# DoeringChristian/mitsuba3-experiments

Measured on AMD Instinct MI355X. Metric: Mpaths/sec on bedroom@1280×720 spp=256, 1/2/4/8 GPUs; HBM GB/s vs peak, higher is better.
Workload: dtype f32; 1 GPU; path-mis.py NEE+MIS (BASELINE configs[1]) on bedroom-proxy 1280x720, global spp=256 split over 1 rank(s) by sample range, max_depth=8, rr_depth=2; global_spp=256, spp_per_rank=256, parallelism=sample-range shards x1

## Files before the change

mitsuba3-experiments_amd/csrc/device_common.h:

```cpp
#pragma once
#include <hip/hip_runtime.h>

#include "mtx_core/bsdf.h"
#include "mtx_core/geometry.h"
#include "mtx_core/interaction.h"
#include "mtx_core/rng.h"
#include "wavefront.h"

namespace mtxd {

using namespace mtx;

inline size_t stack_bytes(const DevScene &s) {
  const size_t a = s.stack_entries, b = 2 * (size_t)s.occ_stack_entries;
  return (a > b ? a : b) * sizeof(uint32_t) * kTraceBlock;
}
inline size_t persistent_stack_bytes(const DevScene &s, bool occ) {
  return occ ? (size_t)s.occ_lds_entries * kTraceBlock * sizeof(uint2) + (size_t)s.occ_lds_top * 80
             : (size_t)s.lds_entries * kTraceBlock * sizeof(int32_t) + (size_t)s.lds_top * 64;
}

__device__ __forceinline__ SceneView make_view(const DevScene &s) {
  SceneView v;
  v.nodes = reinterpret_cast<const int32_t *>(s.nodes);
// ... 102 lines not shown
__device__ __forceinline__ uint32_t wave_append(uint32_t *counter, bool pred) {
  const uint64_t mask = __ballot(pred);
  const uint32_t prefix =
      __builtin_amdgcn_mbcnt_hi((uint32_t)(mask >> 32), __builtin_amdgcn_mbcnt_lo((uint32_t)mask, 0u));
  const uint32_t total = (uint32_t)__popcll(mask);
  uint32_t base = 0;
  if (total) {
    const uint32_t leader = (uint32_t)(__ffsll((unsigned long long)mask) - 1);
    if (lane_id() == leader) base = atomicAdd(counter, total);
    base = __builtin_amdgcn_readlane(base, leader);
  }
  return base + prefix;
}

template <int BLOCK>
__device__ __forceinline__ uint32_t block_reserve(uint32_t cnt, uint32_t *counter) {
  constexpr int W = BLOCK / 64;
  __shared__ uint32_t wsum[W];
  __shared__ uint32_t bbase;
  const uint32_t wave = threadIdx.x >> 6, lane = threadIdx.x & 63;
  uint32_t x = cnt;
#pragma unroll
  for (int off = 1; off < 64; off <<= 1) {
    const uint32_t y = __shfl_up(x, off);
    if (lane >= (uint32_t)off) x += y;
  }
  if (lane == 63) wsum[wave] = x;
  __syncthreads();
  if (threadIdx.x == 0) {
    uint32_t t = 0;
#pragma unroll
    for (int w = 0; w < W; ++w) {
      const uint32_t v = wsum[w];
      wsum[w] = t;
      t += v;
    }
    bbase = t ? atomicAdd(counter, t) : 0u;
  }
  __syncthreads();
  const uint32_t r = bbase + wsum[wave] + x - cnt;
  __syncthreads();
  return r;
}

template <int BLOCK>
__device__ __forceinline__ void block_append2(bool p0, bool p1, bool p1_hi, uint32_t *c, uint32_t parity,
                                              uint32_t &s0, uint32_t &s1) {
  constexpr int W = BLOCK / 64;
  __shared__ uint32_t wcnt[2][3][W];
  __shared__ uint32_t bbase[2][3];
  const uint32_t wave = threadIdx.x >> 6, lane = threadIdx.x & 63;
  const uint64_t m0 = __ballot(p0), ml = __ballot(p1 && !p1_hi), mh = __ballot(p1 && p1_hi);
  if (lane == 0) {
    wcnt[parity][0][wave] = (uint32_t)__popcll(m0);
    wcnt[parity][1][wave] = (uint32_t)__popcll(ml);
    wcnt[parity][2][wave] = (uint32_t)__popcll(mh);
  }
  __syncthreads();
  if (threadIdx.x == 0) {
    uint32_t t0 = 0, tl = 0, th = 0;
#pragma unroll
    for (int w = 0; w < W; ++w) {
      t0 += wcnt[parity][0][w];
      tl += wcnt[parity][1][w];
      th += wcnt[parity][2][w];
    }
    uint64_t base = 0;
    if (t0 | tl | th)
      base = atomicAdd(reinterpret_cast<unsigned long long *>(c), ((unsigned long long)(tl + th) << 32) | t0);
    bbase[parity][0] = (uint32_t)base;
    bbase[parity][1] = (uint32_t)(base >> 32);
    bbase[parity][2] = (uint32_t)(base >> 32) + tl;
  }
  __syncthreads();
  uint32_t o0 = bbase[parity][0], ol = bbase[parity][1], oh = bbase[parity][2];
  for (uint32_t w = 0; w < wave; ++w) {
    o0 += wcnt[parity][0][w];
    ol += wcnt[parity][1][w];
    oh += wcnt[parity][2][w];
  }
  s0 = o0 + __builtin_amdgcn_mbcnt_hi((uint32_t)(m0 >> 32), __builtin_amdgcn_mbcnt_lo((uint32_t)m0, 0u));
  s1 = p1_hi ? oh + __builtin_amdgcn_mbcnt_hi((uint32_t)(mh >> 32), __builtin_amdgcn_mbcnt_lo((uint32_t)mh, 0u))
             : ol + __builtin_amdgcn_mbcnt_hi((uint32_t)(ml >> 32), __builtin_amdgcn_mbcnt_lo((uint32_t)ml, 0u));
}

__device__ __forceinline__ unsigned long long wave_sum_u64(unsigned long long v) {
  for (int off = 32; off > 0; off >>= 1) v += __shfl_xor(v, off);
  return v;
}


__device__ __forceinline__ void lds_node64(const int4 *top, int32_t node, int4 &a, int4 &rf, int4 &qa, int2 &qb) {
  typedef int v4i __attribute__((ext_vector_type(4)));
  typedef int v2i __attribute__((ext_vector_type(2)));
  v4i x0, x1, x2;
  v2i x3;
  const uint32_t la = (uint32_t)(uintptr_t)(const __attribute__((address_space(3))) char *)top + 64u * (uint32_t)node;
  asm volatile(
      "ds_read_b128 %0, %4\n\t"
      "ds_read_b128 %1, %4 offset:16\n\t"
      "ds_read_b128 %2, %4 offset:32\n\t"
      "ds_read_b64 %3, %4 offset:48\n\t"
      "s_waitcnt lgkmcnt(0)"
      : "=&v"(x0), "=&v"(x1), "=&v"(x2), "=&v"(x3)
      : "v"(la));
  a = make_int4(x0.x, x0.y, x0.z, x0.w);
  rf = make_int4(x1.x, x1.y, x1.z, x1.w);
  qa = make_int4(x2.x, x2.y, x2.z, x2.w);
  qb = make_int2(x3.x, x3.y);
}

__device__ __forceinline__ int wide_visit_regs(const TraceRay &r, int4 a, int4 rf, int4 qa, int2 qb, float tbest,
                                               int32_t c[4], uint32_t *key_out = nullptr) {
  uint32_t key[4];
  const uint32_t eb = (uint32_t)a.w;
  const int n = wide_node_keys_e(r, __int_as_float(a.x), __int_as_float(a.y), __int_as_float(a.z),
                                 (int)(int8_t)(uint8_t)(eb & 0xffu), (int)(int8_t)(uint8_t)((eb >> 8) & 0xffu),
                                 (int)(int8_t)(uint8_t)((eb >> 16) & 0xffu), (int)(eb >> 24), (uint32_t)qa.x,
                                 (uint32_t)qa.y, (uint32_t)qa.z, (uint32_t)qa.w, (uint32_t)qb.x, (uint32_t)qb.y,
                                 tbest, key);
  c[0] = rf.x;
  c[1] = rf.y;
  c[2] = rf.z;
  c[3] = rf.w;
#define MTX_CAS2(i, j)                         \
  {                                            \
    const bool sw_ = key[j] < key[i];          \
    const uint32_t ki_ = key[i], kj_ = key[j]; \
    const int32_t ci_ = c[i], cj_ = c[j];      \
    key[i] = sw_ ? kj_ : ki_;                  \
    key[j] = sw_ ? ki_ : kj_;                  \
    c[i] = sw_ ? cj_ : ci_;                    \
    c[j] = sw_ ? ci_ : cj_;                    \
  }
  MTX_CAS2(0, 1) MTX_CAS2(2, 3) MTX_CAS2(0, 2) MTX_CAS2(1, 3) MTX_CAS2(1, 2)
#undef MTX_CAS2
  if (key_out) {
#pragma unroll
    for (int k = 0; k < 4; ++k) key_out[k] = key[k];
  }
  return n;
}

__device__ __forceinline__ int wide_visit(const DevScene &s, const TraceRay &r, int32_t node, float tbest,
                                          int32_t c[4], const int4 *top = nullptr, int top_n = 0,
                                          uint32_t *key_out = nullptr) {
  int4 a, rf, qa;
  int2 qb;
  if (node < top_n) {
    lds_node64(top, node, a, rf, qa, qb);
  } else {
    const int4 *np = s.nodes + 4 * node;
    a = np[0];
    rf = np[1];
    qa = np[2];
    qb = *reinterpret_cast<const int2 *>(np + 3);
  }
  return wide_visit_regs(r, a, rf, qa, qb, tbest, c, key_out);
}

__device__ __forceinline__ void traverse_closest(const DevScene &s, int32_t *stk, const TraceRay &r, float &tbest,
                                                 uint32_t &prim_best, float &bu, float &bv, uint32_t &nv,
                                                 uint32_t &tv) {
  int sp = 0;
  int32_t node = 0;
  while (true) {
// ... 452 lines not shown
```

mitsuba3-experiments_amd/csrc/kernels.hip:

```cpp
#include <hip/hip_runtime.h>

#include <algorithm>

#include "device_common.h"
#include "mtx_core/film.h"
#include "restir_dev.h"

using namespace mtx;

#ifndef MTX_SHADE_MIN_BLOCKS
#define MTX_SHADE_MIN_BLOCKS 3
#endif
constexpr int kShadeMinBlocks = MTX_SHADE_MIN_BLOCKS;

namespace mtxd {

struct ClosestSrc {
  using Payload = uint32_t;
  WaveBuffers b;
  const uint32_t *queue;
  const float4 *ro, *rd;
  __device__ __forceinline__ void load(uint32_t k, TraceRay &r, float &tmax, uint32_t &payload) const {
    const float4 o4 = ld_stream<kNtTrace>(ro + k), d4 = ld_stream<kNtTrace>(rd + k);
    r = make_trace_ray(V3{o4.x, o4.y, o4.z}, V3{d4.x, d4.y, d4.z}, o4.w);
    tmax = o4.w;
    payload = k;
  }
  __device__ __forceinline__ void finish(uint32_t slot, bool, float t, uint32_t prim, float u, float v) const {
    st_stream<kNtTraceSt>(b.hit + slot, make_float4(prim == 0xffffffffu ? kInf : t, __uint_as_float(prim), u, v));
  }
};

#define MTX_TRACE_ATTR __attribute__((amdgpu_waves_per_eu(8)))
#ifndef MTX_CLOSEST_WAVES
#define MTX_CLOSEST_WAVES 8
#endif
template <bool STATS>
__global__ __launch_bounds__(kTraceBlock) __attribute__((amdgpu_waves_per_eu(MTX_CLOSEST_WAVES))) void k_trace_closest(DevScene s, WaveBuffers b, uint32_t bounce) {
  const uint32_t rp = (bounce + b.ray_par) & 1u;
  const ClosestSrc src{b, b.queue[bounce & 1], b.ray_o[rp], b.ray_d[rp]};
  uint32_t nv = 0, tv = 0, nr = 0, wi[2] = {0, 0};
  trace_loop<false, STATS>(s, src, b.counters[4 * bounce + 0], b.xheads + (2 * bounce) * kXSlotWords, nv, tv, nr,
                           wi);
  if (STATS) {
    unsigned long long a = wave_sum_u64(nv), c = wave_sum_u64(tv), n = wave_sum_u64(nr);
    unsigned long long w0 = wave_sum_u64(wi[0]), w1 = wave_sum_u64(wi[1]);
    if ((threadIdx.x & 63) == 0 && n) {
      atomicAdd(&b.stats[0], a);
      atomicAdd(&b.stats[1], c);
      atomicAdd(&b.stats[4], n);
      atomicAdd(&b.stats[6], w0);
      atomicAdd(&b.stats[7], w1);
    }
  }
}

__device__ __forceinline__ void apply_shadow(float4 &L, float4 rt, float4 rx, bool occluded) {
  const uint32_t fl = __float_as_uint(rt.w);
  if (!occluded) {
    if (fl & 1u) {
      L.x = fmaf(rt.x, rx.x, L.x);
      L.y = fmaf(rt.y, rx.y, L.y);
      L.z = fmaf(rt.z, rx.z, L.z);
    } else {
      L.x = L.x + rx.x;
      L.y = L.y + rx.y;
      L.z = L.z + rx.z;
    }
  } else {
    const float qnan = __uint_as_float(0x7fc00000u);
    if (fl & 2u) L.x = qnan;
    if (fl & 4u) L.y = qnan;
    if (fl & 8u) L.z = qnan;
  }
}

constexpr uint32_t kShadowFinal = 16u;

struct ShadowSrc {
  struct Payload {
    uint32_t k, li;
    float4 t;
    float lw;
  };
  WaveBuffers b;
  __device__ __forceinline__ void load(uint32_t k, TraceRay &r, float &tmax, Payload &pl) const {
    const float4 o4 = ld_stream<kNtTrace>(&b.shadow[k].o), d4 = ld_stream<kNtTrace>(&b.shadow[k].d);
    r = make_trace_ray(V3{o4.x, o4.y, o4.z}, V3{d4.x, d4.y, d4.z}, o4.w);
    tmax = o4.w;
    pl.k = k;
    pl.li = __float_as_uint(d4.w);
    pl.t = ld_stream<kNtTrace>(&b.shadow[k].t);
    pl.lw = b.shadow[k].x.w;
  }
  __device__ __forceinline__ void finish(const Payload &pl, bool occluded, float, uint32_t, float, float) const {
    const uint32_t fl = __float_as_uint(pl.t.w);
    if (!(fl & kShadowFinal)) {
      if (occluded && (fl & 14u) == 0u) return;
      float4 L = b.L[0][pl.li];
      apply_shadow(L, pl.t, b.shadow[pl.k].x, occluded);
      b.L[0][pl.li] = L;
      return;
    }
    if (!occluded) {
      st_stream<kNtTraceSt>(b.L[0] + pl.li, make_float4(pl.t.x, pl.t.y, pl.t.z, pl.lw));
    } else if (fl & 14u) {
      float4 L = b.shadow[pl.k].x;
      const float qnan = __uint_as_float(0x7fc00000u);
      if (fl & 2u) L.x = qnan;
      if (fl & 4u) L.y = qnan;
      if (fl & 8u) L.z = qnan;
      b.L[0][pl.li] = L;
    }
  }
};

template <bool STATS>
__global__ __launch_bounds__(kTraceBlock) MTX_TRACE_ATTR void k_trace_shadow(DevScene s, WaveBuffers b, uint32_t bounce) {
  const ShadowSrc src{b};
  uint32_t nv = 0, tv = 0, nr = 0;
  trace_loop<true>(s, src, b.counters[4 * (bounce + 1) + 1], b.xheads + (2 * bounce + 1) * kXSlotWords, nv, tv, nr);
  if (STATS) {
    unsigned long long a = wave_sum_u64(nv), c = wave_sum_u64(tv), n = wave_sum_u64(nr);
    if ((threadIdx.x & 63) == 0 && n) {
      atomicAdd(&b.stats[2], a);
      atomicAdd(&b.stats[3], c);
      atomicAdd(&b.stats[5], n);
    }
  }
}

__device__ __forceinline__ void init_path(const WaveBuffers &b, const ChunkParams &p, uint32_t i, const Ray &ray,
                                          const Pcg32 &rng, float2 pos, bool env) {
  uint32_t depth = 0, flags = 0;
  if (p.integrator == MTX_INT_PATH_MIS) {
    depth = 0;
    flags = PF_PREV_DELTA | (env ? PF_VALID_RAY : 0u);
  } else if (p.integrator == MTX_INT_SIMPLE) {
    depth = 0;
  } else {
    depth = 1;
  }
  st_stream<kNtRaygen>(b.ray_o[0] + i, make_float4(ray.o.x, ray.o.y, ray.o.z, ray.maxt));
  st_stream<kNtRaygen>(b.ray_d[0] + i, make_float4(ray.d.x, ray.d.y, ray.d.z, 0.f));
  st_stream<kNtRaygen>(b.misc[0] + i,
                       make_uint4((uint32_t)rng.state, (uint32_t)(rng.state >> 32), rng.seq, depth | (flags << 16)));
  b.pos[i] = pos;
  if (!p.ident0) b.queue[0][i] = i;
}

__global__ void k_raygen_camera(DevScene s, WaveBuffers b, ChunkParams p) {
  const uint32_t i = blockIdx.x * blockDim.x + threadIdx.x;
  if (i == 0) b.counters[0] = p.n_paths;
  if (i >= p.n_paths) return;
  const uint32_t px_local = i / p.spp, smp = i - px_local * p.spp;
  const uint32_t pix = p.px0 + px_local;
  const uint32_t y = pix / p.width, x = pix - y * p.width;
  const uint32_t lane = pix * p.spp_total + p.sample_offset + smp;
  Pcg32 rng = sampler_lane(p.seed, lane);
  const V2 u = rng.next_2d();
  const float sx = (float)x + u.x, sy = (float)y + u.y;
  const V2 adj = V2{sx / (float)p.width, sy / (float)p.height};
  const Ray ray = camera_ray(s.camera, adj);
  init_path(b, p, i, ray, rng, make_float2(sx, sy), s.has_env != 0);
}

__global__ void k_raygen_rays(DevScene s, WaveBuffers b, ChunkParams p, const float *rays, const uint32_t *lanes,
                              uint32_t rng_skip) {
  const uint32_t i = blockIdx.x * blockDim.x + threadIdx.x;
  if (i == 0) b.counters[0] = p.n_paths;
  if (i >= p.n_paths) return;
  Pcg32 rng = sampler_lane(p.seed, lanes[i]);
  for (uint32_t k = 0; k < rng_skip; ++k) rng.next_u32();
  const float *r = rays + 6 * (size_t)i;
  Ray ray{V3{r[0], r[1], r[2]}, V3{r[3], r[4], r[5]}, kLargest};
  init_path(b, p, i, ray, rng, make_float2(0.f, 0.f), s.has_env != 0);
}

#define kInitThr make_float4(1.f, 1.f, 1.f, 1.f)
#define kInitL make_float4(0.f, 0.f, 0.f, 1.f)
#define kInitPrev make_float4(0.f, 0.f, 0.f, 0.f)

#ifndef MTX_DIAG_STAMPS
#define MTX_DIAG_STAMPS 0
#endif
constexpr int kStampSegs = 8;
struct Stamps {
  unsigned long long prev, acc[kStampSegs];
};
#if MTX_DIAG_STAMPS
__device__ unsigned long long g_shade_stamps[kStampSegs + 2];
#define MTX_STAMP(st, i)                                                                  \
  do {                                                                                    \
    unsigned long long t_;                                                                \
    __builtin_amdgcn_sched_barrier(0);                                                    \
    asm volatile("s_memtime %0\n\ts_waitcnt lgkmcnt(0)" : "=s"(t_)::"memory");          \
    __builtin_amdgcn_sched_barrier(0);                                                    \
    (st).acc[i] += t_ - (st).prev;                                                        \
    (st).prev = t_;                                                                       \
  } while (0)
#endif

struct ShadeIO {
  ShadowRec rec;
  bool emit;
  bool em_hi;
  bool query;
  float4 qp, qd, qt;
  float4 nro, nrd, nthr, nprev;
  float4 nL;
  uint4 nmisc;
  float warm;
#if MTX_DIAG_STAMPS
  Stamps st;
#endif
};

constexpr bool shadow_final_form(int INT) {
  return INT == MTX_INT_PATH || INT == MTX_INT_PATH_MIS || INT == MTX_INT_NRC || INT == MTX_INT_PSSMLT_PATH;
}
constexpr bool shadow_rmw_form(int INT) { return INT == MTX_INT_NERAD_RHS; }

template <int INT, bool FINAL>
__device__ __forceinline__ void make_shadow(ShadeIO &io, const SurfaceInteraction &si, const DirectionSample &ds,
                                            V3 T, V3 X, V3 Xo, bool fma_form, const V3 *Lcur = nullptr) {
  static_assert(FINAL ? shadow_final_form(INT) : shadow_rmw_form(INT),
                "shadow record form does not match where this integrator's L is stored (shadow_final_form)");
  uint32_t fl = fma_form ? 1u : 0u;
  bool vis_noop, occ_noop;
  if (fma_form) {
    fl |= (Xo.x == 0.f && isfinite_(T.x)) ? 0u : 2u;
    fl |= (Xo.y == 0.f && isfinite_(T.y)) ? 0u : 4u;
    fl |= (Xo.z == 0.f && isfinite_(T.z)) ? 0u : 8u;
    vis_noop = X.x == 0.f && X.y == 0.f && X.z == 0.f && isfinite_(T.x) && isfinite_(T.y) && isfinite_(T.z);
  } else {
    fl |= (Xo.x == 0.f) ? 0u : 2u;
    fl |= (Xo.y == 0.f) ? 0u : 4u;
    fl |= (Xo.z == 0.f) ? 0u : 8u;
    vis_noop = X.x == 0.f && X.y == 0.f && X.z == 0.f;
  }
  occ_noop = (fl & 14u) == 0u;
  io.emit = !(vis_noop && occ_noop);
  if (!io.emit) return;
  io.em_hi = (ds.emitter & 1) != 0;
  const Ray sr = spawn_ray_to(si.p, si.n, ds.p);
  io.rec.o = make_float4(sr.o.x, sr.o.y, sr.o.z, sr.maxt);
  io.rec.d = make_float4(sr.d.x, sr.d.y, sr.d.z, 0.f);
  if constexpr (FINAL) {
    float4 lv = make_float4(Lcur->x, Lcur->y, Lcur->z, 0.f);
    apply_shadow(lv, make_float4(T.x, T.y, T.z, __uint_as_float(fl)), make_float4(X.x, X.y, X.z, 0.f), false);
    io.rec.t = make_float4(lv.x, lv.y, lv.z, __uint_as_float(fl | kShadowFinal));
    io.rec.x = make_float4(Lcur->x, Lcur->y, Lcur->z, 0.f);
  } else {
    io.rec.t = make_float4(T.x, T.y, T.z, __uint_as_float(fl));
    io.rec.x = make_float4(X.x, X.y, X.z, 0.f);
  }
}

__device__ __forceinline__ void apply_shadow_rec(float4 &L, const ShadowRec &rec, bool occluded) {
  const uint32_t fl = __float_as_uint(rec.t.w);
  if (!(fl & kShadowFinal)) {
    apply_shadow(L, rec.t, rec.x, occluded);
  } else if (!occluded) {
    L = make_float4(rec.t.x, rec.t.y, rec.t.z, L.w);
  } else {
    const float qnan = __uint_as_float(0x7fc00000u);
    if (fl & 2u) L.x = qnan;
    if (fl & 4u) L.y = qnan;
    if (fl & 8u) L.z = qnan;
// ... 446 lines not shown
  const V3 ray_d = V3{rd.x, rd.y, rd.z};
  const SurfaceInteraction si = compute_si_dev(s, h.x, __float_as_uint(h.y), h.z, h.w, ray_d);
  io.emit = false;
  io.query = false;
  V3 L = V3{Lr.x, Lr.y, Lr.z};
  V3 f = V3{th.x, th.y, th.z};
  V3 f2 = V3{pv.x, pv.y, pv.z};
  if (RENDER && bounce == 0) {
    f = v3s(1.f);
    f2 = v3s(1.f);
    depth = 0;
  }
  if (!RENDER && bounce == 0) {
    const mtx_material mat = sv.materials[si.material];
    DirectionSample ds;
    const V3 em = sample_emitter_direction(sv, si.p, rng.next_2d(), &ds);
    V3 val;
    float pdf;
    bsdf_eval_pdf(sv.bsdf, mat, si.uv, si.wi, to_local(si.sh, ds.d), &val, &pdf);
    const float mis = mis_weight_b(ds.pdf, pdf);
    make_shadow<MTX_INT_NERAD_RHS, false>(io, si, ds, v3s(1.f), val * mis * em, val * mis * v3s(0.f), false);
    const float s1 = rng.next_1d();
    const V2 s2 = rng.next_2d();
    BSDFSample bs;
    const V3 w = bsdf_sample(sv.bsdf, mat, si.uv, si.wi, s1, s2, &bs);
    const Ray nray = spawn_ray(si.p, si.n, to_world(si.sh, bs.wo));
    io.nro = make_float4(nray.o.x, nray.o.y, nray.o.z, nray.maxt);
    io.nrd = make_float4(nray.d.x, nray.d.y, nray.d.z, 0.f);
    b.thr[0][path] = make_float4(w.x, w.y, w.z, 1.f);
    b.L[kFinal][path] = make_float4(L.x, L.y, L.z, bs.pdf);
    b.prev[0][path] = make_float4(si.p.x, si.p.y, si.p.z, 0.f);
    b.misc[kFinal][path] = make_uint4((uint32_t)rng.state, (uint32_t)(rng.state >> 32), rng.seq, 0u);
    return true;
  }
  if (!RENDER && bounce == 1) {
    const V3 prev_p = f2;
    const V3 rel = si.p - prev_p;
    const float dist = norm(rel);
    const float em_pdf = pdf_emitter_direction(sv, si.emitter, rel / dist, dist, si.sh.n);
    f = f * mis_weight_b(Lr.w, em_pdf);
    f2 = v3s(1.f);
  }
  BSDFSample bs;
  bs.type = 0;
  V3 w = v3s(0.f);
  const float s1 = rng.next_1d();
  const V2 s2 = rng.next_2d();
  if (si.valid) {
    const mtx_material mat = sv.materials[si.material];
    w = bsdf_sample(sv.bsdf, mat, si.uv, si.wi, s1, s2, &bs);
  }
  if (bounce > (RENDER ? 0u : 1u)) depth += 1;
  const bool chain = (bs.type & BF_DELTA) != 0 && depth < 10;
  if (chain) {
    f2 = f2 * w;
    const Ray nray = spawn_ray(si.p, si.n, to_world(si.sh, bs.wo));
    io.nro = make_float4(nray.o.x, nray.o.y, nray.o.z, nray.maxt);
    io.nrd = make_float4(nray.d.x, nray.d.y, nray.d.z, 0.f);
    b.thr[0][path] = make_float4(f.x, f.y, f.z, 1.f);
    b.prev[0][path] = make_float4(f2.x, f2.y, f2.z, 0.f);
    b.misc[kFinal][path] = make_uint4((uint32_t)rng.state, (uint32_t)(rng.state >> 32), rng.seq, depth);
    return true;
  }
  f = f * f2;
  if (!si.valid) f = f * 0.f;
  const V3 le = emitter_eval(sv, si.emitter, si.wi);
  if (RENDER && !si.valid) {
    L = v3s(0.f) * f + le;
    b.L[kFinal][path] = make_float4(L.x, L.y, L.z, Lr.w);
  } else if (si.valid) {
    io.query = true;
    const V3 wi = to_world(si.sh, si.wi);
    io.qp = make_float4(si.p.x, si.p.y, si.p.z, 0.f);
    io.qd = make_float4(wi.x, wi.y, wi.z, 0.f);
    io.qt = make_float4(f.x, f.y, f.z, __uint_as_float(path));
    b.prev[0][path] = make_float4(le.x, le.y, le.z, 0.f);
  } else {
    L = L + f * (le + v3s(0.f));
    b.L[kFinal][path] = make_float4(L.x, L.y, L.z, Lr.w);
  }
  return false;
}

template <int INT>
__global__ __launch_bounds__(kShadeBlock, kShadeMinBlocks) void k_shade(DevScene s, WaveBuffers b, ChunkParams p, uint32_t bounce) {
  const SceneView sv = make_view(s);
  const uint32_t count = b.counters[4 * bounce + 0];
  const uint32_t *in_q = b.queue[bounce & 1];
  uint32_t *out_q = b.queue[(bounce + 1) & 1];
  uint32_t *out_cnt = &b.counters[4 * (bounce + 1) + 0];
  const uint32_t rp = (bounce + b.ray_par) & 1u;
  constexpr bool kNerad = INT == MTX_INT_NERAD_RHS || INT == MTX_INT_NERAD;
  const uint32_t stride = gridDim.x * kShadeBlock;
  uint32_t parity = 0;
  uint32_t path = 0;
  float4 h = make_float4(0.f, 0.f, 0.f, 0.f);
  const bool ident = bounce == 0 && p.ident0;
  if (blockIdx.x * kShadeBlock + threadIdx.x < count) {
    const uint32_t i0 = blockIdx.x * kShadeBlock + threadIdx.x;
    path = ident ? i0 : ld_stream<kNtQueue>(in_q + i0);
    h = ld_stream<kNtShade>(b.hit + i0);
  }

#if MTX_DIAG_STAMPS
  Stamps stp{};
  unsigned long long steps = 0;
  asm volatile("s_memtime %0\n\ts_waitcnt lgkmcnt(0)" : "=s"(stp.prev)::"memory");
#endif
  for (uint32_t base = blockIdx.x * kShadeBlock; base < count; base += stride, parity ^= 1u) {
    const uint32_t i = base + threadIdx.x;
    const uint32_t inext = i + stride;
    uint32_t path_n = 0;
    if (inext < count) path_n = ident ? inext : ld_stream<kNtQueue>(in_q + inext);
#if MTX_SHADE_WARM
    float4 hn = make_float4(0.f, 0.f, 0.f, 0.f);
    if (inext < count) hn = b.hit[inext];
    const uint32_t pn = __float_as_uint(hn.y);
    const float4 *wp = (inext < count && pn != 0xffffffffu) ? s.shade_rec + 8 * (size_t)pn : nullptr;
#else
    const float4 *wp = nullptr;
#endif
    ShadeIO io;
    io.emit = false;
    io.em_hi = false;
    io.query = false;
    io.warm = 0.f;
#if MTX_DIAG_STAMPS
    ++steps;
    MTX_STAMP(stp, 0);
    io.st = stp;
#endif
    bool cont = false;
    const bool valid = i < count;
    if (valid) {
      if constexpr (INT == MTX_INT_PSSMLT_SIMPLE)
        cont = shade_pssmlt(s, sv, b, p, bounce, path, i, h, io);
      else if constexpr (INT == MTX_INT_SIMPLE)
        cont = shade_simple(s, sv, b, p, bounce, path, i, h, io);
      else if constexpr (INT == MTX_INT_PSSMLT_PATH)
        cont = shade_pssmlt_path(s, sv, b, p, bounce, path, i, h, io);
      else if constexpr (INT == MTX_INT_NERAD_RHS)
        cont = shade_nerad<false>(s, sv, b, bounce, path, i, h, io);
      else if constexpr (INT == MTX_INT_NERAD)
        cont = shade_nerad<true>(s, sv, b, bounce, path, i, h, io);
      else
        cont = shade_path<INT>(s, sv, b, p, bounce, path, i, h, io, wp);
    }
    (void)wp;
    const uint32_t path_c = path;
    path = path_n;
#if MTX_SHADE_WARM
    h = hn;
    asm volatile("" ::"v"(io.warm));
#else
    if (inext < count) h = ld_stream<kNtShade>(b.hit + inext);
#endif

#if MTX_DIAG_STAMPS
    stp = io.st;
#endif
    uint32_t slot, sslot;
    block_append2<kShadeBlock>(cont, io.emit, io.emit && io.em_hi, out_cnt, parity, slot, sslot);
    if (cont) {
      st_stream<kNtQueue>(out_q + slot, path_c);
      st_stream<kNtShadeSt>(b.ray_o[rp ^ 1u] + slot, io.nro);
      st_stream<kNtShadeSt>(b.ray_d[rp ^ 1u] + slot, io.nrd);
      if constexpr (!kNerad) st_stream<kNtShadeSt>(b.thr[rp ^ 1u] + slot, io.nthr);
      if constexpr (INT == MTX_INT_PATH_MIS || INT == MTX_INT_PATH || INT == MTX_INT_NRC || INT == MTX_INT_PSSMLT_PATH)
        st_stream<kNtShadeSt>(b.prev[rp ^ 1u] + slot, io.nprev);
      if constexpr (!kNerad) {
        st_stream<kNtShadeSt>(b.L[rp ^ 1u] + slot, io.nL);
        st_stream<kNtShadeSt>(b.misc[rp ^ 1u] + slot, io.nmisc);
      }
    } else if (!kNerad && valid) {
      st_stream<kNtShadeSt>(b.L[kFinal] + path_c, io.nL);
      if (!p.drop_end_misc) st_stream<kNtShadeSt>(b.misc[kFinal] + path_c, io.nmisc);
    }
    if (io.emit) {
      const uint32_t li = (kNerad || !cont) ? kFinal * b.capacity + path_c : (rp ^ 1u) * b.capacity + slot;
      io.rec.d.w = __uint_as_float(li);
      if constexpr (!kNerad) io.rec.x.w = io.nL.w;
      ShadowRec *sr = b.shadow + sslot;
      st_stream<kNtShadeSt>(&sr->o, io.rec.o);
      st_stream<kNtShadeSt>(&sr->d, io.rec.d);
      st_stream<kNtShadeSt>(&sr->t, io.rec.t);
      st_stream<kNtShadeSt>(&sr->x, io.rec.x);
    }
#if MTX_DIAG_STAMPS
    MTX_STAMP(stp, 6);
#endif
    if constexpr (INT == MTX_INT_NRC || INT == MTX_INT_NERAD_RHS || INT == MTX_INT_NERAD) {
      if (INT != MTX_INT_NRC || p.nrc_cache) {
        const uint32_t q = block_reserve<kShadeBlock>(io.query ? 1u : 0u, b.cq_count);
        if (io.query) {
          b.cq_p[q] = io.qp;
          b.cq_d[q] = io.qd;
          b.cq_t[q] = io.qt;
        }
      }
    }
#if MTX_DIAG_STAMPS
    MTX_STAMP(stp, 7);
#endif
  }
#if MTX_DIAG_STAMPS
  if ((threadIdx.x & 63u) == 0) {
    for (int k = 0; k < kStampSegs; ++k) atomicAdd(&g_shade_stamps[k], stp.acc[k]);
    atomicAdd(&g_shade_stamps[kStampSegs], steps);
    atomicAdd(&g_shade_stamps[kStampSegs + 1], 1ull);
  }
#endif
}

__global__ void k_flush_tail(WaveBuffers b, uint32_t bounce, uint32_t integrator) {
  const uint32_t n = b.counters[4 * bounce];
  const uint32_t *q = b.queue[bounce & 1];
  const uint32_t rp = (bounce + b.ray_par) & 1u;
  for (uint32_t k = blockIdx.x * blockDim.x + threadIdx.x; k < n; k += gridDim.x * blockDim.x) {
    const uint32_t path = q[k];
    float4 L = b.L[rp][k];
    const uint4 m = b.misc[rp][k];
    if (integrator == MTX_INT_PATH_MIS || integrator == MTX_INT_RESTIR_GI) L.w = end_w(m.w >> 16, L.w);
    b.L[kFinal][path] = L;
    b.misc[kFinal][path] = m;
  }
}

#ifndef MTX_MEGA_MIN_BLOCKS
#define MTX_MEGA_MIN_BLOCKS 3
#endif
static_assert(kShadeBlock == kTraceBlock, "k_path_mega: stack column stride must equal the block width");
#ifndef MTX_MEGA_REFILL
#define MTX_MEGA_REFILL 16
#endif
template <int INT>
__global__ __launch_bounds__(kShadeBlock, MTX_MEGA_MIN_BLOCKS) void k_path_mega(DevScene s, WaveBuffers b, ChunkParams p) {
  static_assert(INT == MTX_INT_PATH_MIS || INT == MTX_INT_PATH, "megakernel: path / path-mis only");
  extern __shared__ int4 mega_lds[];
  const SceneView sv = make_view(s);
  const uint32_t count = b.counters[0];
  const uint32_t iters = p.max_depth > 1u ? p.max_depth : 1u;
  int32_t *stk = reinterpret_cast<int32_t *>(mega_lds) + threadIdx.x;
  uint32_t *ostk = reinterpret_cast<uint32_t *>(mega_lds) + threadIdx.x;
  const uint32_t lane = threadIdx.x & 63u;
  bool has = false, drained = false;
  uint32_t qi = 0, path = 0, bounce = 0;
  while (true) {
    if (!drained) {
      const uint64_t idle = __ballot(!has);
      const uint32_t n_idle = (uint32_t)__popcll(idle);
      if (n_idle >= MTX_MEGA_REFILL || idle == ~0ull) {
        const uint32_t leader = (uint32_t)(__ffsll((unsigned long long)idle) - 1);
        uint32_t base = 0;
        if (lane == leader) base = atomicAdd(&b.counters[2], n_idle);
        base = __builtin_amdgcn_readlane(base, leader);
        if (base + n_idle >= count) drained = true;
        const uint32_t rk = __builtin_amdgcn_mbcnt_hi((uint32_t)(idle >> 32), __builtin_amdgcn_mbcnt_lo((uint32_t)idle, 0u));
        if (!has && base + rk < count) {
          has = true;
          qi = base + rk;
          path = p.ident0 ? qi : b.queue[0][qi];
          bounce = 0;
        }
      }
    }
    if (__ballot(has) == 0) break;
    if (has) {
      const uint32_t rp = (bounce + b.ray_par) & 1u;
      const float4 o4 = b.ray_o[rp][qi], d4 = b.ray_d[rp][qi];
      const TraceRay r = make_trace_ray(V3{o4.x, o4.y, o4.z}, V3{d4.x, d4.y, d4.z}, o4.w);
      float tbest = o4.w, bu = 0.f, bv = 0.f;
      uint32_t prim = 0xffffffffu, nv = 0, tv = 0;
      traverse_closest(s, stk, r, tbest, prim, bu, bv, nv, tv);
      const float4 h = make_float4(prim == 0xffffffffu ? kInf : tbest, __uint_as_float(prim), bu, bv);
      ShadeIO io;
      io.emit = false;
      io.em_hi = false;
      io.query = false;
      const bool cont = shade_path<INT>(s, sv, b, p, bounce, path, qi, h, io);
      if (io.emit) {
        const float4 so = io.rec.o, sd = io.rec.d;
        const TraceRay sr = make_trace_ray(V3{so.x, so.y, so.z}, V3{sd.x, sd.y, sd.z}, so.w);
        apply_shadow_rec(io.nL, io.rec, traverse_occ(s, ostk, sr, so.w, nv, tv));
      }
      ++bounce;
      if (cont && bounce < iters) {
// ... 677 lines not shown
```

mitsuba3-experiments_amd/csrc/wavefront.h:

```cpp
#pragma once
#include <hip/hip_runtime.h>
#include <stdint.h>

#include "mtx.h"
#include "mtx_core/nerad.h"

namespace mtxd {

enum : uint32_t {
  PF_VALID_RAY = 1u,
  PF_PREV_DELTA = 2u,
  PF_PRIMARY_VALID = 4u,
  PF_CACHE_QUERY = 8u,
};

#ifndef MTX_TRACE_BLOCK
#define MTX_TRACE_BLOCK 256
#endif
constexpr int kTraceBlock = MTX_TRACE_BLOCK;
constexpr int kShadeBlock = 256;
constexpr uint32_t kLdsStack = 16;
constexpr uint32_t kOccLdsStack = 8;
#ifndef MTX_LDS_TOP
#define MTX_LDS_TOP 64
#endif
#ifndef MTX_OCC_LDS_TOP
#define MTX_OCC_LDS_TOP 48
#endif
#ifndef MTX_SHADE_WARM
#define MTX_SHADE_WARM 1
#endif
#ifndef MTX_CACHE_SORT
#define MTX_CACHE_SORT 2
#endif
#ifndef MTX_ENCODE_LM
#define MTX_ENCODE_LM 1
#endif
#ifndef MTX_STREAMS
#define MTX_STREAMS 2
#endif

constexpr uint32_t kXcds = 8;
constexpr uint32_t kXHeadStride = 32;
constexpr uint32_t kXSlotWords = kXcds * kXHeadStride;

struct DevScene {
  const int4 *nodes;
  const float *tri;
  const int4 *occ_nodes;
  const float *occ_tri;
  const uint32_t *tri_vidx;
  const uint32_t *tri_shape;
  const float *vpos;
  const float *vnormal;
  const float *vuv;
  const mtx_shape *shapes;
  const float4 *shade_rec;
  const mtx_material *materials;
  const mtx_emitter *emitters;
  const mtx_texture *textures;
  const float *texels;
  const float *tables;
  uint32_t n_tris, n_emitters;
  uint32_t stack_entries;
  uint32_t lds_entries;
  uint32_t lds_top;
  uint32_t occ_stack_entries, occ_lds_entries, occ_lds_top;
  uint32_t trace_batch;
  void *stack_ovf;
  uint32_t ovf_threads;
  uint32_t urefill;
  uint32_t occ_urefill;
  uint32_t xcd_claim;
  mtx_camera camera;
  uint32_t has_env;
  float env_radiance[3], env_center[3], env_radius;
};

inline size_t stack_ovf_bytes(const DevScene &s) {
  const size_t a = (size_t)(s.stack_entries - s.lds_entries) * sizeof(int32_t);
  const size_t b = (size_t)(s.occ_stack_entries - s.occ_lds_entries) * sizeof(uint2);
  const size_t n = (a > b ? a : b) * s.ovf_threads;
  return n > 8 ? n : 8;
}

constexpr int kFinal = 2;

struct ShadowRec {
  float4 o;
  float4 d;
  float4 t;
  float4 x;
};

struct WaveBuffers {
  float4 *ray_o[2], *ray_d[2];
  uint32_t ray_par;
  float4 *thr[2], *prev[2];
  float4 *L[3];
  uint4 *misc[3];
  float2 *pos;
  float4 *hit;
  uint32_t *queue[2];
  ShadowRec *shadow;
  uint32_t *counters;
  uint32_t *xheads;
  unsigned long long *stats;
  uint32_t capacity;
  float4 *mlt_cur;
  float4 *mlt_L;
  float2 *mlt_prop;
  float4 *vpath;
  float4 *vprop;
// ... 104 lines not shown
```

Before: 1456 Mpaths/s.

## Split shadow records into SoA planes and add an optional deferred LDS-staged shade append

Shadow-ray records move from an array of 64-byte structs to separate float4 planes, with a macro defaulting to on. In plane mode the fourth word is no longer stored, and the final unoccluded store writes only RGB, which saves bandwidth and makes per-lane accesses contiguous. A second option, off by default, stages continuing-path state and shadow records in LDS. It publishes them one iteration late with a single atomic per block, to spread the global stores away from the append. That path adds extra barriers and LDS use, and plane mode depends on L already holding the right value when the x word is gone.

After: 1473 Mpaths/s (median of 6 runs). 1.2% higher.

```diff
diff --git a/mitsuba3-experiments_amd/csrc/device_common.h b/mitsuba3-experiments_amd/csrc/device_common.h
--- a/mitsuba3-experiments_amd/csrc/device_common.h
+++ b/mitsuba3-experiments_amd/csrc/device_common.h
@@ -208,6 +208,21 @@
   s0 = o0 + __builtin_amdgcn_mbcnt_hi((uint32_t)(m0 >> 32), __builtin_amdgcn_mbcnt_lo((uint32_t)m0, 0u));
   s1 = p1_hi ? oh + __builtin_amdgcn_mbcnt_hi((uint32_t)(mh >> 32), __builtin_amdgcn_mbcnt_lo((uint32_t)mh, 0u))
              : ol + __builtin_amdgcn_mbcnt_hi((uint32_t)(ml >> 32), __builtin_amdgcn_mbcnt_lo((uint32_t)ml, 0u));
+}
+
+constexpr int kShadowWords = MTX_SHADOW_PLANES ? 3 : 4;
+template <int BLOCK>
+struct ShadeStage {
+  float4 st[6][BLOCK];
+  float4 sh[kShadowWords][BLOCK];
+  uint32_t path[BLOCK];
+  uint32_t wcnt[3][BLOCK / 64];
+  uint32_t pub[4];
+};
+template <int BLOCK>
+__device__ __forceinline__ ShadeStage<BLOCK> &shade_stage() {
+  __shared__ ShadeStage<BLOCK> sg;
+  return sg;
 }
 
 __device__ __forceinline__ unsigned long long wave_sum_u64(unsigned long long v) {
diff --git a/mitsuba3-experiments_amd/csrc/kernels.hip b/mitsuba3-experiments_amd/csrc/kernels.hip
--- a/mitsuba3-experiments_amd/csrc/kernels.hip
+++ b/mitsuba3-experiments_amd/csrc/kernels.hip
@@ -76,36 +76,56 @@
 }
 
 constexpr uint32_t kShadowFinal = 16u;
+__device__ __forceinline__ float4 *shadow_word(const WaveBuffers &b, uint32_t g, uint32_t k) {
+#if MTX_SHADOW_PLANES
+  return reinterpret_cast<float4 *>(b.shadow) + ((size_t)g * b.capacity + k);
+#else
+  return reinterpret_cast<float4 *>(b.shadow + k) + g;
+#endif
+}
 
 struct ShadowSrc {
   struct Payload {
     uint32_t k, li;
     float4 t;
+#if !MTX_SHADOW_PLANES
     float lw;
+#endif
   };
   WaveBuffers b;
   __device__ __forceinline__ void load(uint32_t k, TraceRay &r, float &tmax, Payload &pl) const {
-    const float4 o4 = ld_stream<kNtTrace>(&b.shadow[k].o), d4 = ld_stream<kNtTrace>(&b.shadow[k].d);
+    const float4 o4 = ld_stream<kNtTrace>(shadow_word(b, 0, k)), d4 = ld_stream<kNtTrace>(shadow_word(b, 1, k));
     r = make_trace_ray(V3{o4.x, o4.y, o4.z}, V3{d4.x, d4.y, d4.z}, o4.w);
     tmax = o4.w;
     pl.k = k;
     pl.li = __float_as_uint(d4.w);
-    pl.t = ld_stream<kNtTrace>(&b.shadow[k].t);
-    pl.lw = b.shadow[k].x.w;
+    pl.t = ld_stream<kNtTrace>(shadow_word(b, 2, k));
+#if !MTX_SHADOW_PLANES
+    pl.lw = shadow_word(b, 3, k)->w;
+#endif
   }
   __device__ __forceinline__ void finish(const Payload &pl, bool occluded, float, uint32_t, float, float) const {
     const uint32_t fl = __float_as_uint(pl.t.w);
     if (!(fl & kShadowFinal)) {
       if (occluded && (fl & 14u) == 0u) return;
       float4 L = b.L[0][pl.li];
-      apply_shadow(L, pl.t, b.shadow[pl.k].x, occluded);
+      apply_shadow(L, pl.t, *shadow_word(b, 3, pl.k), occluded);
       b.L[0][pl.li] = L;
       return;
     }
     if (!occluded) {
+#if MTX_SHADOW_PLANES
+      typedef float v3f __attribute__((ext_vector_type(3)));
+      *reinterpret_cast<v3f *>(b.L[0] + pl.li) = v3f{pl.t.x, pl.t.y, pl.t.z};
+#else
       st_stream<kNtTraceSt>(b.L[0] + pl.li, make_float4(pl.t.x, pl.t.y, pl.t.z, pl.lw));
+#endif
     } else if (fl & 14u) {
-      float4 L = b.shadow[pl.k].x;
+#if MTX_SHADOW_PLANES
+      float4 L = b.L[0][pl.li];
+#else
+      float4 L = *shadow_word(b, 3, pl.k);
+#endif
       const float qnan = __uint_as_float(0x7fc00000u);
       if (fl & 2u) L.x = qnan;
       if (fl & 4u) L.y = qnan;
@@ -184,7 +204,7 @@
 #ifndef MTX_DIAG_STAMPS
 #define MTX_DIAG_STAMPS 0
 #endif
-constexpr int kStampSegs = 8;
+constexpr int kStampSegs = 10;
 struct Stamps {
   unsigned long long prev, acc[kStampSegs];
 };
@@ -797,6 +817,40 @@
   return false;
 }
 
+constexpr uint32_t kShadowStaged = 32u;
+template <int INT>
+__device__ __forceinline__ void shade_flush(const WaveBuffers &b, const ShadeStage<kShadeBlock> &sg, uint32_t *out_q,
+                                            uint32_t np) {
+  static_assert(shadow_final_form(INT), "the deferred append stages the state planes k_shade stores for these");
+  const uint32_t tid = threadIdx.x;
+  const uint32_t b0 = sg.pub[0], b1 = sg.pub[1], n0 = sg.pub[2], ns = sg.pub[3];
+  if (tid < n0) {
+    const uint32_t slot = b0 + tid;
+    st_stream<kNtQueue>(out_q + slot, sg.path[tid]);
+    st_stream<kNtShadeSt>(b.ray_o[np] + slot, sg.st[0][tid]);
+    st_stream<kNtShadeSt>(b.ray_d[np] + slot, sg.st[1][tid]);
+    st_stream<kNtShadeSt>(b.thr[np] + slot, sg.st[2][tid]);
+    st_stream<kNtShadeSt>(b.prev[np] + slot, sg.st[3][tid]);
+    st_stream<kNtShadeSt>(b.L[np] + slot, sg.st[4][tid]);
+    const float4 m = sg.st[5][tid];
+    st_stream<kNtShadeSt>(b.misc[np] + slot, make_uint4(__float_as_uint(m.x), __float_as_uint(m.y),
+                                                        __float_as_uint(m.z), __float_as_uint(m.w)));
+  }
+  if (tid < ns) {
+    float4 d = sg.sh[1][tid], t = sg.sh[2][tid];
+    const uint32_t fl = __float_as_uint(t.w);
+    if (fl & kShadowStaged) {
+      d.w = __uint_as_float(np * b.capacity + b0 + __float_as_uint(d.w));
+      t.w = __uint_as_float(fl & ~kShadowStaged);
+    }
+    const uint32_t k = b1 + tid;
+    st_stream<kNtShadeSt>(shadow_word(b, 0, k), sg.sh[0][tid]);
+    st_stream<kNtShadeSt>(shadow_word(b, 1, k), d);
+    st_stream<kNtShadeSt>(shadow_word(b, 2, k), t);
+    if constexpr (!MTX_SHADOW_PLANES) st_stream<kNtShadeSt>(shadow_word(b, 3, k), sg.sh[kShadowWords - 1][tid]);
+  }
+}
+
 template <int INT>
 __global__ __launch_bounds__(kShadeBlock, kShadeMinBlocks) void k_shade(DevScene s, WaveBuffers b, ChunkParams p, uint32_t bounce) {
   const SceneView sv = make_view(s);
@@ -808,6 +862,15 @@
   constexpr bool kNerad = INT == MTX_INT_NERAD_RHS || INT == MTX_INT_NERAD;
   const uint32_t stride = gridDim.x * kShadeBlock;
   uint32_t parity = 0;
+  constexpr bool kDefer = MTX_SHADE_DEFER != 0 && shadow_final_form(INT);
+  unsigned long long pend = 0;
+  if constexpr (kDefer) {
+    if (threadIdx.x == 0) {
+      ShadeStage<kShadeBlock> &sg = shade_stage<kShadeBlock>();
+      sg.pub[2] = 0u;
+      sg.pub[3] = 0u;
+    }
+  }
   uint32_t path = 0;
   float4 h = make_float4(0.f, 0.f, 0.f, 0.f);
   const bool ident = bounce == 0 && p.ident0;
@@ -867,6 +930,7 @@
 #if MTX_SHADE_WARM
     h = hn;
     asm volatile("" ::"v"(io.warm));
+    if constexpr (kDefer) asm volatile("" ::"v"(path), "v"(h.y), "v"(h.z), "v"(h.w));
 #else
     if (inext < count) h = ld_stream<kNtShade>(b.hit + inext);
 #endif
@@ -874,35 +938,125 @@
 #if MTX_DIAG_STAMPS
     stp = io.st;
 #endif
-    uint32_t slot, sslot;
-    block_append2<kShadeBlock>(cont, io.emit, io.emit && io.em_hi, out_cnt, parity, slot, sslot);
-    if (cont) {
-      st_stream<kNtQueue>(out_q + slot, path_c);
-      st_stream<kNtShadeSt>(b.ray_o[rp ^ 1u] + slot, io.nro);
-      st_stream<kNtShadeSt>(b.ray_d[rp ^ 1u] + slot, io.nrd);
-      if constexpr (!kNerad) st_stream<kNtShadeSt>(b.thr[rp ^ 1u] + slot, io.nthr);
-      if constexpr (INT == MTX_INT_PATH_MIS || INT == MTX_INT_PATH || INT == MTX_INT_NRC || INT == MTX_INT_PSSMLT_PATH)
-        st_stream<kNtShadeSt>(b.prev[rp ^ 1u] + slot, io.nprev);
-      if constexpr (!kNerad) {
-        st_stream<kNtShadeSt>(b.L[rp ^ 1u] + slot, io.nL);
-        st_stream<kNtShadeSt>(b.misc[rp ^ 1u] + slot, io.nmisc);
-      }
-    } else if (!kNerad && valid) {
-      st_stream<kNtShadeSt>(b.L[kFinal] + path_c, io.nL);
-      if (!p.drop_end_misc) st_stream<kNtShadeSt>(b.misc[kFinal] + path_c, io.nmisc);
-    }
-    if (io.emit) {
-      const uint32_t li = (kNerad || !cont) ? kFinal * b.capacity + path_c : (rp ^ 1u) * b.capacity + slot;
-      io.rec.d.w = __uint_as_float(li);
-      if constexpr (!kNerad) io.rec.x.w = io.nL.w;
-      ShadowRec *sr = b.shadow + sslot;
-      st_stream<kNtShadeSt>(&sr->o, io.rec.o);
-      st_stream<kNtShadeSt>(&sr->d, io.rec.d);
-      st_stream<kNtShadeSt>(&sr->t, io.rec.t);
-      st_stream<kNtShadeSt>(&sr->x, io.rec.x);
-    }
+    if constexpr (kDefer) {
+      ShadeStage<kShadeBlock> &sg = shade_stage<kShadeBlock>();
+      constexpr uint32_t W = kShadeBlock / 64;
+      const uint32_t wave = threadIdx.x >> 6, lane = threadIdx.x & 63;
+      const bool em_lo = io.emit && !io.em_hi, em_hi = io.emit && io.em_hi;
+      const uint64_t m0 = __ballot(cont), ml = __ballot(em_lo), mh = __ballot(em_hi);
+      if (lane == 0) {
+        sg.wcnt[0][wave] = (uint32_t)__popcll(m0);
+        sg.wcnt[1][wave] = (uint32_t)__popcll(ml);
+        sg.wcnt[2][wave] = (uint32_t)__popcll(mh);
+      }
+      if (!cont && valid) {
+        st_stream<kNtShadeSt>(b.L[kFinal] + path_c, io.nL);
+        if (!p.drop_end_misc) st_stream<kNtShadeSt>(b.misc[kFinal] + path_c, io.nmisc);
+      }
+      if (threadIdx.x == 0) {
+        sg.pub[0] = (uint32_t)pend;
+        sg.pub[1] = (uint32_t)(pend >> 32);
+      }
+      __syncthreads();
 #if MTX_DIAG_STAMPS
-    MTX_STAMP(stp, 6);
+      MTX_STAMP(stp, 6);
+#endif
+      shade_flush<INT>(b, sg, out_q, rp ^ 1u);
+      uint32_t o0 = 0, ol = 0, oh = 0, t0 = 0, tl = 0, th = 0;
+#pragma unroll
+      for (uint32_t w = 0; w < W; ++w) {
+        const uint32_t c0 = sg.wcnt[0][w], cl = sg.wcnt[1][w], ch = sg.wcnt[2][w];
+        if (w < wave) {
+          o0 += c0;
+          ol += cl;
+          oh += ch;
+        }
+        t0 += c0;
+        tl += cl;
+        th += ch;
+      }
+      const uint32_t l0 = o0 + __builtin_amdgcn_mbcnt_hi((uint32_t)(m0 >> 32), __builtin_amdgcn_mbcnt_lo((uint32_t)m0, 0u));
+      const uint32_t ls =
+          io.em_hi ? tl + oh + __builtin_amdgcn_mbcnt_hi((uint32_t)(mh >> 32), __builtin_amdgcn_mbcnt_lo((uint32_t)mh, 0u))
+                   : ol + __builtin_amdgcn_mbcnt_hi((uint32_t)(ml >> 32), __builtin_amdgcn_mbcnt_lo((uint32_t)ml, 0u));
+#if MTX_DIAG_STAMPS
+      MTX_STAMP(stp, 8);
+#endif
+      __syncthreads();
+      if (cont) {
+        sg.path[l0] = path_c;
+        sg.st[0][l0] = io.nro;
+        sg.st[1][l0] = io.nrd;
+        sg.st[2][l0] = io.nthr;
+        sg.st[3][l0] = io.nprev;
+        sg.st[4][l0] = io.nL;
+        sg.st[5][l0] = make_float4(__uint_as_float(io.nmisc.x), __uint_as_float(io.nmisc.y),
+                                   __uint_as_float(io.nmisc.z), __uint_as_float(io.nmisc.w));
+      }
+      if (io.emit) {
+        uint32_t fl = __float_as_uint(io.rec.t.w);
+        if (cont) {
+          io.rec.d.w = __uint_as_float(l0);
+          fl |= kShadowStaged;
+        } else {
+          io.rec.d.w = __uint_as_float(kFinal * b.capacity + path_c);
+        }
+        io.rec.t.w = __uint_as_float(fl);
+        sg.sh[0][ls] = io.rec.o;
+        sg.sh[1][ls] = io.rec.d;
+        sg.sh[2][ls] = io.rec.t;
+        if constexpr (!MTX_SHADOW_PLANES) {
+          io.rec.x.w = io.nL.w;
+          sg.sh[kShadowWords - 1][ls] = io.rec.x;
+        }
+      }
+      if (threadIdx.x == 0) {
+        if (t0 | tl | th) {
+          typedef __attribute__((address_space(1))) unsigned long long gu64;
+          gu64 *cp = (gu64 *)reinterpret_cast<unsigned long long *>(out_cnt);
+          asm volatile("" : "+v"(cp));
+          pend = __hip_atomic_fetch_add(cp, ((unsigned long long)(tl + th) << 32) | t0, __ATOMIC_RELAXED,
+                                        __HIP_MEMORY_SCOPE_AGENT);
+        }
+        sg.pub[2] = t0;
+        sg.pub[3] = tl + th;
+      }
+    } else {
+      uint32_t slot, sslot;
+      block_append2<kShadeBlock>(cont, io.emit, io.emit && io.em_hi, out_cnt, parity, slot, sslot);
+#if MTX_DIAG_STAMPS
+      MTX_STAMP(stp, 6);
+#endif
+      if (cont) {
+        st_stream<kNtQueue>(out_q + slot, path_c);
+        st_stream<kNtShadeSt>(b.ray_o[rp ^ 1u] + slot, io.nro);
+        st_stream<kNtShadeSt>(b.ray_d[rp ^ 1u] + slot, io.nrd);
+        if constexpr (!kNerad) st_stream<kNtShadeSt>(b.thr[rp ^ 1u] + slot, io.nthr);
+        if constexpr (INT == MTX_INT_PATH_MIS || INT == MTX_INT_PATH || INT == MTX_INT_NRC || INT == MTX_INT_PSSMLT_PATH)
+          st_stream<kNtShadeSt>(b.prev[rp ^ 1u] + slot, io.nprev);
+        if constexpr (!kNerad) {
+          st_stream<kNtShadeSt>(b.L[rp ^ 1u] + slot, io.nL);
+          st_stream<kNtShadeSt>(b.misc[rp ^ 1u] + slot, io.nmisc);
+        }
+      } else if (!kNerad && valid) {
+        st_stream<kNtShadeSt>(b.L[kFinal] + path_c, io.nL);
+        if (!p.drop_end_misc) st_stream<kNtShadeSt>(b.misc[kFinal] + path_c, io.nmisc);
+      }
+      if (io.emit) {
+        const uint32_t li = (kNerad || !cont) ? kFinal * b.capacity + path_c : (rp ^ 1u) * b.capacity + slot;
+        io.rec.d.w = __uint_as_float(li);
+        if constexpr (!kNerad) io.rec.x.w = io.nL.w;
+        st_stream<kNtShadeSt>(shadow_word(b, 0, sslot), io.rec.o);
+        st_stream<kNtShadeSt>(shadow_word(b, 1, sslot), io.rec.d);
+        st_stream<kNtShadeSt>(shadow_word(b, 2, sslot), io.rec.t);
+        if constexpr (kNerad || !MTX_SHADOW_PLANES) st_stream<kNtShadeSt>(shadow_word(b, 3, sslot), io.rec.x);
+      }
+#if MTX_DIAG_STAMPS
+      MTX_STAMP(stp, 8);
+#endif
+    }
+#if MTX_DIAG_STAMPS
+    MTX_STAMP(stp, 9);
 #endif
     if constexpr (INT == MTX_INT_NRC || INT == MTX_INT_NERAD_RHS || INT == MTX_INT_NERAD) {
       if (INT != MTX_INT_NRC || p.nrc_cache) {
@@ -917,6 +1071,15 @@
 #if MTX_DIAG_STAMPS
     MTX_STAMP(stp, 7);
 #endif
+  }
+  if constexpr (kDefer) {
+    ShadeStage<kShadeBlock> &sg = shade_stage<kShadeBlock>();
+    if (threadIdx.x == 0) {
+      sg.pub[0] = (uint32_t)pend;
+      sg.pub[1] = (uint32_t)(pend >> 32);
+    }
+    __syncthreads();
+    shade_flush<INT>(b, sg, out_q, rp ^ 1u);
   }
 #if MTX_DIAG_STAMPS
   if ((threadIdx.x & 63u) == 0) {
diff --git a/mitsuba3-experiments_amd/csrc/wavefront.h b/mitsuba3-experiments_amd/csrc/wavefront.h
--- a/mitsuba3-experiments_amd/csrc/wavefront.h
+++ b/mitsuba3-experiments_amd/csrc/wavefront.h
@@ -29,6 +29,12 @@
 #endif
 #ifndef MTX_SHADE_WARM
 #define MTX_SHADE_WARM 1
+#endif
+#ifndef MTX_SHADE_DEFER
+#define MTX_SHADE_DEFER 0
+#endif
+#ifndef MTX_SHADOW_PLANES
+#define MTX_SHADOW_PLANES 1
 #endif
 #ifndef MTX_CACHE_SORT
 #define MTX_CACHE_SORT 2
```
